# stcodeer/Frequency-wised_All-in-One_Image_Restoration_Model

Hardware: AMD Instinct MI355X
Metric: training images/sec @128x128 (higher is better)
Workload: dtype bf16; 1 GPU; BASELINE configs[1]: Uformer encoder+decoder (all_3_bands, L=3, freq MSA), denoise sigma=25, 128x128, phase-2 train step (fwd+bwd+Adam, DropPath on); per_gpu_batch=16, global_batch=16, parallelism=dp1, hip_graph=True

## Files before the change

### frequency-wised_all-in-one_image_restoration_model_amd/csrc/fw_elem.hip

```cpp
#include "fw_common.h"
#include <stdlib.h>

namespace {

constexpr int TPB = 256;
FW_DEV long gtid() { return (long)blockIdx.x * TPB + threadIdx.x; }
FW_DEV long gstride() { return (long)gridDim.x * TPB; }
static inline int grid_for(long n, int cap = 8192) { long g = (n + TPB - 1) / TPB; return (int)(g < 1 ? 1 : (g > cap ? cap : g)); }

template <typename T> FW_DEV void ldvec(const T* p, float* f) {
    unpack16<T>(*reinterpret_cast<const uint4*>(p), f);
}
template <typename T> FW_DEV void stvec(T* p, const float* f) { *reinterpret_cast<uint4*>(p) = pack16<T>(f); }
template <typename T> FW_DEV void ldvec4(const T* p, float* f);
template <> FW_SPEC void ldvec4<float>(const float* p, float* f) { unpack16<float>(*reinterpret_cast<const uint4*>(p), f); }
template <> FW_SPEC void ldvec4<bf16raw>(const bf16raw* p, float* f) {
    const uint2 v = *reinterpret_cast<const uint2*>(p);
    f[0] = __uint_as_float(v.x << 16); f[1] = __uint_as_float(v.x & 0xffff0000u);
    f[2] = __uint_as_float(v.y << 16); f[3] = __uint_as_float(v.y & 0xffff0000u);
}
template <typename T> FW_DEV void stvec4(T* p, const float* f);
template <> FW_SPEC void stvec4<float>(float* p, const float* f) { *reinterpret_cast<uint4*>(p) = pack16<float>(f); }
template <> FW_SPEC void stvec4<bf16raw>(bf16raw* p, const float* f) {
    *reinterpret_cast<uint2*>(p) = make_uint2(pack_bf2(f[0], f[1]), pack_bf2(f[2], f[3]));
}

template <typename T>
__global__ void cast_rows_kernel(const float* __restrict__ src, long lds_, T* __restrict__ dst, long ldd, long rows, int cols,
                                 const float* __restrict__ rowscale, int rps) {
    const int c4n = cols >> 2;
    for (long i = gtid(); i < rows * c4n; i += gstride()) {
        const long r = i / c4n; const int c = (int)(i % c4n) * 4;
        const f32x4 v = *reinterpret_cast<const f32x4*>(src + r * lds_ + c);
        const float s = rowscale ? rowscale[r / rps] : 1.f;
        T* d = dst + r * ldd + c;
        if (sizeof(T) == 4) *reinterpret_cast<f32x4*>(d) = v * s;
        else *reinterpret_cast<uint2*>(d) = make_uint2(pack_bf2(v[0] * s, v[1] * s), pack_bf2(v[2] * s, v[3] * s));
    }
}
__global__ void copy_rows_kernel(const float* __restrict__ src, long lds_, float* __restrict__ dst, long ldd, long rows, int cols, int acc) {
    const int c4n = cols >> 2;
    for (long i = gtid(); i < rows * c4n; i += gstride()) {
        const long r = i / c4n; const int c = (int)(i % c4n) * 4;
        f32x4 v = *reinterpret_cast<const f32x4*>(src + r * lds_ + c);
        if (acc) v += *reinterpret_cast<const f32x4*>(dst + r * ldd + c);
        *reinterpret_cast<f32x4*>(dst + r * ldd + c) = v;
    }
}
template <typename T>
__global__ void add_rows_kernel(const T* __restrict__ src, long lds_, T* __restrict__ dst, long ldd, long rows, int cols) {
    const int c4n = cols >> 2;
    for (long i = gtid(); i < rows * c4n; i += gstride()) {
        const long r = i / c4n; const int c = (int)(i % c4n) * 4;
        for (int e = 0; e < 4; ++e) {
// ... 917 lines not shown
        const int s = i & 3, l = (i >> 2) & 63, nt = (i >> 8) & 1, ch = i >> 9;
        const int k = ch * 16 + 4 * (l >> 4) + s, n = nt * 16 + (l & 15);
        sm[i] = (k < C && n < 27) ? w[((long)(n / 9) * C + k) * 9 + n % 9] : 0.f;
    }
    __syncthreads();
    const int l = lane_id(), wave = threadIdx.x >> 6;
    const EcTiles T(B, H, W);
    for (long t = blockIdx.x; t < T.n; t += gridDim.x) {
        long b; int y0, x0;
        T.at(t, b, y0, x0);
        for (int grp = wave; grp < (EC_PLANE + 15) / 16; grp += 4) {
            int r = grp * 16 + (l & 15); r = r < EC_PLANE ? r : EC_PLANE - 1;
            const int y = y0 + r / EC_PW - 1, x = x0 + r % EC_PW - 1;
            const bool ok = y >= 0 && y < H && x >= 0 && x < W;
            const int yc = y < 0 ? 0 : (y >= H ? H - 1 : y), xc = x < 0 ? 0 : (x >= W ? W - 1 : x);
            const float* row = fea + ((b * H + yc) * W + xc) * ldf;
            f32x4 acc0 = f32x4{0.f, 0.f, 0.f, 0.f}, acc1 = acc0;
            for (int c0 = 0; c0 < KC; c0 += 4) {
                uint4 af[4];
#pragma unroll
                for (int j = 0; j < 4; ++j) {
                    const int k = (c0 + j) * 16 + 4 * (l >> 4);
                    af[j] = *reinterpret_cast<const uint4*>(row + (k < C ? k : 0));
                }
#pragma unroll
                for (int j = 0; j < 4; ++j) {
                    const int k = (c0 + j) * 16 + 4 * (l >> 4);
                    if (!(ok && k < C)) af[j] = make_uint4(0u, 0u, 0u, 0u);
                    const int ch = c0 + j < KC ? c0 + j : KC - 1;
                    mma_chunk<float>(acc0, af[j], wl[(ch * 2 + 0) * 64 + l]);
                    mma_chunk<float>(acc1, af[j], wl[(ch * 2 + 1) * 64 + l]);
                }
            }
            float* pd = prod + (grp * 16 + 4 * (l >> 4)) * OP_PS + (l & 15);
#pragma unroll
            for (int rr = 0; rr < 4; ++rr) { pd[rr * OP_PS] = acc0[rr]; pd[rr * OP_PS + 16] = acc1[rr]; }
        }
        __syncthreads();
        for (int i = threadIdx.x; i < 3 * EC_PIX; i += 256) {
            const int co = i / EC_PIX, p = i % EC_PIX, ty = p / EC_TX, tx = p % EC_TX, y = y0 + ty, x = x0 + tx;
            const float* pp = prod + (ty * EC_PW + tx) * OP_PS + co * 9;
            const long po = ((b * 3 + co) * H + (y < H ? y : H - 1)) * W + (x < W ? x : W - 1);
            float s = bias[co] + (img ? img[po] : 0.f);
#pragma unroll
            for (int ky = 0; ky < 3; ++ky)
#pragma unroll
                for (int kx = 0; kx < 3; ++kx) s += pp[(ky * EC_PW + kx) * OP_PS + ky * 3 + kx];
            if (y < H && x < W) out[po] = s;
        }
        __syncthreads();
    }
}

__global__ void l1_loss_kernel(const float* __restrict__ a, const float* __restrict__ b, float* __restrict__ da, long n, float gscale,
                               float* __restrict__ loss) {
    float s = 0.f;
    for (long i = gtid(); i < n; i += gstride()) {
        const float d = a[i] - b[i];
        s += fabsf(d);
        if (da) da[i] = (d > 0.f ? 1.f : (d < 0.f ? -1.f : 0.f)) * gscale / n;
    }
    s = wave_sum(s);
    if (lane_id() == 0) atomicAdd(loss, s / n);
}
__global__ void ce0_loss_kernel(const float* __restrict__ logits, float* __restrict__ dlogits, int R, int N, float gscale, float* __restrict__ loss) {
    const int r = blockIdx.x;
    const float* x = logits + (long)r * N;
    float mx = -3.0e38f;
    for (int j = threadIdx.x; j < N; j += 64) mx = fmaxf(mx, x[j]);
    mx = wave_max(mx);
    float s = 0.f;
    for (int j = threadIdx.x; j < N; j += 64) s += __expf(x[j] - mx);
    s = wave_sum(s);
    const float lse = mx + __logf(s);
    if (dlogits)
        for (int j = threadIdx.x; j < N; j += 64) dlogits[(long)r * N + j] = (__expf(x[j] - lse) - (j == 0 ? 1.f : 0.f)) * gscale / R;
    if (threadIdx.x == 0) atomicAdd(loss, (lse - x[0]) / R);
}

__global__ void adam_tick_kernel(float* __restrict__ hyper, float b1, float b2) { hyper[1] *= b1; hyper[2] *= b2; hyper[3] += 1.f; }
template <typename T>
__global__ void adam_kernel(float* __restrict__ p, const float* __restrict__ g, float* __restrict__ m, float* __restrict__ v,
                            T* __restrict__ shadow, long n, const float* __restrict__ hyper, float b1, float b2, float eps) {
    const float lr = hyper[0], bc1 = 1.f - hyper[1], bc2_sqrt = sqrtf(1.f - hyper[2]);
    for (long i = gtid(); i < n; i += gstride()) {
        const float gi = g[i];
        const float mi = m[i] * b1 + gi * (1.f - b1);
        const float vi = v[i] * b2 + gi * gi * (1.f - b2);
        m[i] = mi; v[i] = vi;
        const float denom = sqrtf(vi) / bc2_sqrt + eps;
        const float pi = p[i] - (lr / bc1) * (mi / denom);
        p[i] = pi;
        if (shadow) TT<T>::st(shadow + i, pi);
    }
}
template <typename T>
__global__ void ema_kernel(float* __restrict__ pk, const float* __restrict__ pq, T* __restrict__ shadow, long n, float mom) {
    for (long i = gtid(); i < n; i += gstride()) {
        const float x = pk[i] * mom + pq[i] * (1.f - mom);
        pk[i] = x;
        if (shadow) TT<T>::st(shadow + i, x);
    }
}
template <typename T>
__global__ void lrelu_fwd_kernel(const float* __restrict__ x, T* __restrict__ y, long n, float slope) {
    for (long i = gtid(); i < n; i += gstride()) TT<T>::st(y + i, lrelu_f(x[i], slope));
}
template <typename T>
__global__ void lrelu_bwd_kernel(const T* __restrict__ dy, const float* __restrict__ x, float* __restrict__ dx, long n, float slope) {
    for (long i = gtid(); i < n; i += gstride()) dx[i] = TT<T>::ld(dy + i) * (x[i] > 0.f ? 1.f : slope);
}
__global__ __launch_bounds__(256) void slab_reduce_kernel(const float* __restrict__ slab, int nz, long n, long zstride, float* __restrict__ dst,
                                                          int accumulate, int zper, float* __restrict__ dst2, long off2, long n2) {
    __shared__ f32x4 red[3][64];
    const int lane = threadIdx.x & 63, zl = threadIdx.x >> 6;
    const long i4 = (long)blockIdx.x * 64 + lane;
    const long end = dst2 ? off2 + n2 : n;
    const bool live = i4 * 4 < end;
    const int z0 = blockIdx.y * zper, z1 = min(nz, z0 + zper);
    f32x4 s = f32x4{0.f, 0.f, 0.f, 0.f};
    if (live) {
        const float* p = slab + i4 * 4;
        int z = z0 + zl;
        for (; z + 12 < z1; z += 16) {
            const f32x4 a0 = *reinterpret_cast<const f32x4*>(p + (long)z * zstride);
            const f32x4 a1 = *reinterpret_cast<const f32x4*>(p + (long)(z + 4) * zstride);
            const f32x4 a2 = *reinterpret_cast<const f32x4*>(p + (long)(z + 8) * zstride);
            const f32x4 a3 = *reinterpret_cast<const f32x4*>(p + (long)(z + 12) * zstride);
            s += (a0 + a1) + (a2 + a3);
        }
        for (; z < z1; z += 4) s += *reinterpret_cast<const f32x4*>(p + (long)z * zstride);
    }
    if (zl > 0) red[zl - 1][lane] = s;
    __syncthreads();
    if (zl > 0 || !live) return;
    s += red[0][lane] + red[1][lane] + red[2][lane];
    for (int e = 0; e < 4; ++e) {
        const long i = i4 * 4 + e;
        float* d = nullptr;
        if (i < n) d = dst + i;
        else if (dst2 && i >= off2 && i < off2 + n2) d = dst2 + (i - off2);
        if (!d) continue;
        if (gridDim.y > 1) atomicAdd(d, s[e]);
        else if (accumulate) *d += s[e];
        else *d = s[e];
    }
}
__global__ __launch_bounds__(256) void slab_reduce_multi_kernel(const long long* __restrict__ tab, const long long* __restrict__ prefix, int num) {
    int lo = 0, hi = num;
    while (hi - lo > 1) {
        const int mid = (lo + hi) >> 1;
        if (prefix[mid] <= (long long)blockIdx.x) lo = mid; else hi = mid;
    }
    const long long* t = tab + (long)lo * 12;
// ... 241 lines not shown
    if (x_dtype == 1) hipLaunchKernelGGL((colsum_t_kernel<bf16raw>), dim3(grid), dim3(TPB), 0, ST, (const bf16raw*)x, ldx, out, rows, cols, rpb);
    else hipLaunchKernelGGL(colsum_kernel, dim3(grid), dim3(TPB), 0, ST, (const float*)x, ldx, out, rows, cols, rpb);
    FW_LAUNCH_RET();
}
#ifndef FW_EC_WGRAD_CAP
#define FW_EC_WGRAD_CAP 512
#endif
static inline int ec_grid(int B, int H, int W, int cap) {
    const long n = (long)B * ((H + EC_TY - 1) / EC_TY) * ((W + EC_TX - 1) / EC_TX);
    return (int)(n < cap ? n : cap);
}
static inline bool ec_al16(const void* p) { return ((uintptr_t)p & 15) == 0; }
constexpr int OP_PROD_BYTES = ((EC_PLANE + 15) / 16) * 16 * OP_PS * 4;
constexpr int OP_MAX_C = 896;
extern "C" int fw_inproj_fwd(const float* img, const float* w, const float* bias, float* out, long ldo, int B, int H, int W, int C,
                             float slope, void* stream) {
    FW_CHECK_ARG(img && w && bias && out && C % 4 == 0 && ldo % 4 == 0 && C > 0 && C <= 1024 && B > 0 && H > 0 && W > 0);
    FW_CHECK_ARG(ec_al16(out) && ec_al16(bias));
    hipLaunchKernelGGL(edge_conv3_rows_kernel<0>, dim3(ec_grid(B, H, W, 768)), dim3(TPB), 0, ST, img, w, bias, out, ldo, B, H, W, C, slope);
    FW_LAUNCH_RET();
}
extern "C" int fw_inproj_bwd(const float* img, const float* out, long ldo, const float* dy, long ldy, float* dw, float* db, int B,
                             int H, int W, int C, float slope, void* stream) {
    FW_CHECK_ARG(img && out && dy && dw && db && C > 0 && B > 0 && H > 0 && W > 0);
    const dim3 grid(ec_grid(B, H, W, FW_EC_WGRAD_CAP));
    const bool v4 = C % 4 == 0 && ldo % 4 == 0 && ldy % 4 == 0 && ec_al16(out) && ec_al16(dy);
    const int slice = v4 ? 1024 : 256;
    for (int c0 = 0; c0 < C; c0 += slice) {
        const int cs = C - c0 < slice ? C - c0 : slice;
        if (v4) hipLaunchKernelGGL((edge_conv3_wgrad_kernel<4, 0>), grid, dim3(TPB), 0, ST, img, dy + c0, ldy, out + c0, ldo, dw + (long)c0 * 27, db + c0, B, H, W, cs, slope);
        else hipLaunchKernelGGL((edge_conv3_wgrad_kernel<1, 0>), grid, dim3(TPB), 0, ST, img, dy + c0, ldy, out + c0, ldo, dw + (long)c0 * 27, db + c0, B, H, W, cs, slope);
    }
    FW_LAUNCH_RET();
}
extern "C" int fw_outproj_fwd(const float* fea, long ldf, const float* w, const float* bias, const float* img, float* out, int B,
                              int H, int W, int C, void* stream) {
    FW_CHECK_ARG(fea && w && bias && out && C % 4 == 0 && ldf % 4 == 0 && C > 0 && C <= OP_MAX_C && B > 0 && H > 0 && W > 0 && ec_al16(fea));
    const size_t lds = (size_t)((C + 15) / 16) * 2048 + OP_PROD_BYTES;
    FW_SET_LDS_ONCE(outproj_fwd_mfma_kernel, (OP_MAX_C / 16) * 2048 + OP_PROD_BYTES);
    hipLaunchKernelGGL(outproj_fwd_mfma_kernel, dim3(ec_grid(B, H, W, 512)), dim3(TPB), lds, ST, fea, ldf, w, bias, img, out, B, H, W, C);
    FW_LAUNCH_RET();
}
extern "C" int fw_outproj_bwd(const float* dout, const float* fea, long ldf, const float* w, float* dfea, long lddf, float* dw,
                              float* db, int B, int H, int W, int C, void* stream) {
    FW_CHECK_ARG(dout && fea && w && dfea && dw && db && C % 4 == 0 && ldf % 4 == 0 && lddf % 4 == 0 && C > 0 && C <= 1024 && B > 0 && H > 0 && W > 0);
    FW_CHECK_ARG(ec_al16(fea) && ec_al16(dfea));
    hipLaunchKernelGGL(edge_conv3_rows_kernel<1>, dim3(ec_grid(B, H, W, 768)), dim3(TPB), 0, ST, dout, w, (const float*)nullptr, dfea, lddf, B, H, W, C, 0.f);
    hipLaunchKernelGGL((edge_conv3_wgrad_kernel<4, 1>), dim3(ec_grid(B, H, W, FW_EC_WGRAD_CAP)), dim3(TPB), 0, ST, dout, fea, ldf, (const float*)nullptr, 0L, dw, db,
                       B, H, W, C, 0.f);
    FW_LAUNCH_RET();
}
extern "C" int fw_l1_loss(const float* a, const float* b, float* da, long n, float gscale, float* loss, void* stream) {
    FW_CHECK_ARG(a && b && loss && n > 0);
    hipLaunchKernelGGL(l1_loss_kernel, dim3(grid_for(n, 1024)), dim3(TPB), 0, ST, a, b, da, n, gscale, loss);
    FW_LAUNCH_RET();
}
extern "C" int fw_ce0_loss(const float* logits, float* dlogits, int R, int N, float gscale, float* loss, void* stream) {
    FW_CHECK_ARG(logits && loss && R > 0 && N > 0);
    hipLaunchKernelGGL(ce0_loss_kernel, dim3(R), dim3(64), 0, ST, logits, dlogits, R, N, gscale, loss);
    FW_LAUNCH_RET();
}
extern "C" int fw_adam_tick(float* hyper, float b1, float b2, void* stream) {
    FW_CHECK_ARG(hyper);
    hipLaunchKernelGGL(adam_tick_kernel, dim3(1), dim3(1), 0, ST, hyper, b1, b2);
    FW_LAUNCH_RET();
}
extern "C" int fw_adam(int shadow_dtype, float* p, const float* g, float* m, float* v, void* shadow, long n, const float* hyper,
                       float b1, float b2, float eps, void* stream) {
    FW_CHECK_ARG(p && g && m && v && hyper && n > 0);
    if (shadow_dtype == FW_DT_BF16 && shadow) LAUNCH((adam_kernel<bf16raw>), n, p, g, m, v, (bf16raw*)shadow, n, hyper, b1, b2, eps);
    LAUNCH((adam_kernel<float>), n, p, g, m, v, (float*)nullptr, n, hyper, b1, b2, eps);
}
extern "C" int fw_ema(int shadow_dtype, float* pk, const float* pq, void* shadow, long n, float momentum, void* stream) {
    FW_CHECK_ARG(pk && pq && n > 0);
    if (shadow_dtype == FW_DT_BF16 && shadow) LAUNCH((ema_kernel<bf16raw>), n, pk, pq, (bf16raw*)shadow, n, momentum);
    LAUNCH((ema_kernel<float>), n, pk, pq, (float*)nullptr, n, momentum);
}
extern "C" int fw_lrelu_fwd(int dtype, const float* x, void* y, long n, float slope, void* stream) {
    FW_CHECK_ARG(x && y && n > 0);
    if (dtype == FW_DT_BF16) LAUNCH((lrelu_fwd_kernel<bf16raw>), n, x, (bf16raw*)y, n, slope);
    LAUNCH((lrelu_fwd_kernel<float>), n, x, (float*)y, n, slope);
}
extern "C" int fw_lrelu_bwd(int dtype, const void* dy, const float* x, float* dx, long n, float slope, void* stream) {
    FW_CHECK_ARG(dy && x && dx && n > 0);
    if (dtype == FW_DT_BF16) LAUNCH((lrelu_bwd_kernel<bf16raw>), n, (const bf16raw*)dy, x, dx, n, slope);
    LAUNCH((lrelu_bwd_kernel<float>), n, (const float*)dy, x, dx, n, slope);
}
extern "C" int fw_slab_reduce(const float* slab, int nz, long n, long zstride, float* dst, int accumulate, float* dst2, long off2, long n2,
                              void* stream) {
    FW_CHECK_ARG(slab && dst && nz > 0 && n > 0 && zstride % 4 == 0 && ((uintptr_t)slab & 15) == 0);
    FW_CHECK_ARG(!dst2 || (off2 >= n && n2 > 0 && off2 + n2 <= zstride));
    const long end = dst2 ? off2 + n2 : n;
    const long gx = ((end + 3) / 4 + 63) / 64;
    int zper = nz;
    if (accumulate) {
        long splits = 1024 / gx;
        if (splits > nz / 8) splits = nz / 8;
        if (splits < 1) splits = 1;
        zper = (int)((nz + splits - 1) / splits);
    }
    dim3 grid((unsigned)gx, (unsigned)((nz + zper - 1) / zper));
    hipLaunchKernelGGL(slab_reduce_kernel, grid, dim3(256), 0, ST, slab, nz, n, zstride, dst, accumulate, zper, dst2, off2, n2);
    FW_LAUNCH_RET();
}
extern "C" int fw_slab_reduce_multi(const void* tab, const void* prefix, int num, long total_blocks, void* stream) {
    FW_CHECK_ARG(tab && prefix && num > 0 && total_blocks > 0 && total_blocks < (1L << 31));
    hipLaunchKernelGGL(slab_reduce_multi_kernel, dim3((unsigned)total_blocks), dim3(256), 0, ST, (const long long*)tab, (const long long*)prefix, num);
    FW_LAUNCH_RET();
}
extern "C" int fw_permute3_multi(const void* tab, const void* prefix, int num, long total_blocks, void* stream) {
    FW_CHECK_ARG(tab && prefix && num > 0 && total_blocks > 0 && total_blocks < (1L << 31));
    hipLaunchKernelGGL(permute3_multi_kernel, dim3((unsigned)total_blocks), dim3(256), 0, ST, (const long long*)tab, (const long long*)prefix, num);
    FW_LAUNCH_RET();
}
extern "C" int fw_fill(float* p, long n, float v, void* stream) {
    FW_CHECK_ARG(p && n > 0);
    LAUNCH(fill_kernel, n, p, n, v);
}
```

### frequency-wised_all-in-one_image_restoration_model_amd/csrc/fw_heads.hip

```cpp
#include "fw_common.h"

namespace {

template <int N> FW_DEV float block_sum(float v, float* red) {
    v = wave_sum(v);
    __syncthreads();
    if (lane_id() == 0) red[threadIdx.x >> 6] = v;
    __syncthreads();
    float s = 0.f;
    for (int i = 0; i < N / 64; ++i) s += red[i];
    return s;
}

constexpr int DFT_SL = 16, DFT_MAXN = 256;
__global__ __launch_bounds__(256) void dft2_fwd_kernel(const float* __restrict__ img, float* __restrict__ fr, float* __restrict__ fi, int N) {
    __shared__ float hr[DFT_SL * DFT_MAXN], hi[DFT_SL * DFT_MAXN], tc[DFT_MAXN], ts[DFT_MAXN];
    const int rows = N < DFT_SL ? N : DFT_SL;
    const int u0 = blockIdx.y * rows;
    const float* x = img + (size_t)blockIdx.x * N * N;
    for (int k = threadIdx.x; k < N; k += 256) { float sn, cs; sincospif(2.0f * k / N, &sn, &cs); tc[k] = cs; ts[k] = sn; }
    __syncthreads();
    for (int o = threadIdx.x; o < rows * N; o += 256) {
        const int u = u0 + o / N, xx = o % N;
        float ar = 0.f, ai = 0.f;
// ... 357 lines not shown
    float pos = 0.f;
    for (int c = threadIdx.x; c < ED; c += 256) {
        const float a = qq[c] * iq, bb = kk[c] * ik;
        sm[c] = a; khat[((size_t)l * B + b) * ED + c] = bb; pos += a * bb;
    }
    pos = block_sum<256>(pos, red);
    float* lg = logits + ((size_t)l * B + b) * (1 + K);
    if (threadIdx.x == 0) lg[0] = pos * invT;
    const float* Q = queue + (size_t)l * ED * K;
    for (int j = threadIdx.x; j < K; j += 256) {
        float s = 0.f;
        for (int c = 0; c < ED; ++c) s += sm[c] * Q[(size_t)c * K + j];
        lg[1 + j] = s * invT;
    }
}
__global__ __launch_bounds__(256) void moco_logits_bwd_kernel(const float* __restrict__ q, const float* __restrict__ khat, const float* __restrict__ queue,
                                                              const float* __restrict__ dlogits, float* __restrict__ dq, int B, int ED, int K, float invT) {
    __shared__ float red[4];
    const int l = blockIdx.x, b = blockIdx.y;
    const float* qq = q + ((size_t)l * B + b) * ED; const float* kh = khat + ((size_t)l * B + b) * ED;
    const float* dl = dlogits + ((size_t)l * B + b) * (1 + K);
    const float* Q = queue + (size_t)l * ED * K;
    float sq = 0.f;
    for (int c = threadIdx.x; c < ED; c += 256) sq += qq[c] * qq[c];
    sq = block_sum<256>(sq, red);
    const float nq = fmaxf(sqrtf(sq), 1e-12f), iq = 1.f / nq;
    float dot = 0.f;
    float loc[4];
    for (int t = 0; t < 4; ++t) {
        const int c = threadIdx.x + 256 * t;
        loc[t] = 0.f;
        if (c < ED) {
            float s = dl[0] * kh[c];
            for (int j = 0; j < K; ++j) s += dl[1 + j] * Q[(size_t)c * K + j];
            loc[t] = s * invT;
            dot += loc[t] * qq[c] * iq;
        }
    }
    dot = block_sum<256>(dot, red);
    for (int t = 0; t < 4; ++t) {
        const int c = threadIdx.x + 256 * t;
        if (c < ED) dq[((size_t)l * B + b) * ED + c] = (loc[t] - qq[c] * iq * dot) * iq;
    }
}
__global__ void moco_enqueue_kernel(float* __restrict__ queue, const float* __restrict__ khat, long long* __restrict__ ptr, int L, int B, int ED, int K) {
    const int p = (int)*ptr;
    for (int i = blockIdx.x * blockDim.x + threadIdx.x; i < L * B * ED; i += gridDim.x * blockDim.x) {
        const int c = i % ED, b = (i / ED) % B, l = i / (ED * B);
        queue[((size_t)l * ED + c) * K + p + b] = khat[i];
    }
}
__global__ void moco_ptr_kernel(long long* __restrict__ ptr, int B, int K) { *ptr = (*ptr + B) % K; }

constexpr int LFS_MAXT = 1024;
__global__ __launch_bounds__(256) void lfs_xbar_kernel(const float* __restrict__ inter, float* __restrict__ xbar, float* __restrict__ stats, int NT, int C, float eps) {
    __shared__ float mu[LFS_MAXT], rs[LFS_MAXT];
    const size_t blk = (size_t)blockIdx.x;
    const float* x = inter + blk * NT * C;
    const int w = threadIdx.x >> 6, l = lane_id();
    for (int t = w; t < NT; t += 4) {
        float s = 0.f;
        for (int c = l; c < C; c += 64) s += x[(size_t)t * C + c];
        const float m = wave_sum(s) / C;
        float q = 0.f;
        for (int c = l; c < C; c += 64) { const float d = x[(size_t)t * C + c] - m; q += d * d; }
        const float r = rsqrtf(wave_sum(q) / C + eps);
        if (l == 0) { mu[t] = m; rs[t] = r; stats[(blk * NT + t) * 2] = m; stats[(blk * NT + t) * 2 + 1] = r; }
    }
    __syncthreads();
    for (int c = threadIdx.x; c < C; c += 256) {
        float s = 0.f;
        for (int t = 0; t < NT; ++t) s += (x[(size_t)t * C + c] - mu[t]) * rs[t];
        xbar[blk * C + c] = s / NT;
    }
}
__global__ __launch_bounds__(256) void lfs_xbar_bwd_kernel(const float* __restrict__ inter, const float* __restrict__ stats, const float* __restrict__ dxbar,
                                                           float* __restrict__ dinter, int NT, int C) {
    __shared__ float red[4];
    const size_t blk = (size_t)blockIdx.x;
    const float* x = inter + blk * NT * C; float* dx = dinter + blk * NT * C;
    const float* g = dxbar + blk * C;
    float s = 0.f;
    for (int c = threadIdx.x; c < C; c += 256) s += g[c];
    const float m1 = block_sum<256>(s, red) / C / NT;
    const int w = threadIdx.x >> 6, l = lane_id();
    for (int t = w; t < NT; t += 4) {
        const float m = stats[(blk * NT + t) * 2], r = stats[(blk * NT + t) * 2 + 1];
        float q = 0.f;
        for (int c = l; c < C; c += 64) q += g[c] / NT * (x[(size_t)t * C + c] - m) * r;
        const float m2 = wave_sum(q) / C;
        for (int c = l; c < C; c += 64) {
            const float xh = (x[(size_t)t * C + c] - m) * r;
            dx[(size_t)t * C + c] += r * (g[c] / NT - m1 - xh * m2);
        }
    }
}

__global__ __launch_bounds__(64) void lfs_lambda_kernel(const float* __restrict__ xbar, const unsigned long long* __restrict__ ptab,
                                                        const int* __restrict__ heads, const long long* __restrict__ coef_off,
                                                        float* __restrict__ coef, float* __restrict__ save, int B, int C, int nb1) {
    __shared__ float u[16], s1[16], lam[2][16];
    const int blk = blockIdx.x, b = blockIdx.y, h = heads[blk], l = lane_id();
    for (int band = 0; band < nb1; ++band) {
        const unsigned long long* pt = ptab + ((size_t)blk * 2 + band) * 8;
        const float* lnw = (const float*)pt[0]; const float* lnb = (const float*)pt[1];
        const float* W = (const float*)pt[2]; const float* bl = (const float*)pt[3];
        const float* W1 = (const float*)pt[4]; const float* b1 = (const float*)pt[5];
        const float* W2 = (const float*)pt[6]; const float* b2 = (const float*)pt[7];
        const float* xb = xbar + ((size_t)band * B + b) * C;
        for (int hh = 0; hh < h; ++hh) {
            float s = 0.f;
            for (int c = l; c < C; c += 64) s += W[(size_t)hh * C + c] * (lnw[c] * xb[c] + lnb[c]);
            s = wave_sum(s);
            if (l == 0) u[hh] = s + bl[hh];
        }
        __syncthreads();
        float* sv = save + ((((size_t)blk * 2 + band) * B + b) * 16) * 3;
        if (l < h) {
            float a = b1[l];
            for (int j = 0; j < h; ++j) a += W1[l * h + j] * u[j];
            s1[l] = lrelu_f(a, 0.1f);
            sv[l * 3] = u[l]; sv[l * 3 + 1] = a; sv[l * 3 + 2] = s1[l];
        }
        __syncthreads();
        if (l < h) {
            float a = b2[l];
            for (int j = 0; j < h; ++j) a += W2[l * h + j] * s1[j];
            lam[band][l] = a;
        }
        __syncthreads();
    }
    if (l < h) {
        float* cf = coef + coef_off[blk] + ((size_t)b * h + l) * 3;
        if (nb1 == 2) { const float l1 = lam[0][l], l2 = lam[1][l]; cf[0] = 1.f + l2; cf[1] = -l2 * (1.f / 64.f); cf[2] = l1 - l2; }
        else { const float l1 = lam[0][l]; cf[0] = 1.f + l1; cf[1] = -l1 * (1.f / 64.f); cf[2] = 0.f; }
    }
}
__global__ __launch_bounds__(64) void lfs_lambda_bwd_kernel(const float* __restrict__ xbar, const unsigned long long* __restrict__ ptab,
                                                            const unsigned long long* __restrict__ gtab, const int* __restrict__ heads,
                                                            const long long* __restrict__ coef_off, const float* __restrict__ dcoef,
                                                            const float* __restrict__ save, float* __restrict__ dxbar, int B, int C, int nb1) {
    __shared__ float dl[16], da1[16], du[16];
    const int blk = blockIdx.x, b = blockIdx.y, h = heads[blk], l = lane_id();
    for (int band = 0; band < nb1; ++band) {
        const unsigned long long* pt = ptab + ((size_t)blk * 2 + band) * 8;
        const unsigned long long* gt = gtab + ((size_t)blk * 2 + band) * 8;
        const float* lnw = (const float*)pt[0]; const float* lnb = (const float*)pt[1];
// ... 83 lines not shown
    FW_LAUNCH_RET();
}

extern "C" int fw_bn_lrelu_gap_fwd(int dtype, const void* fea, const float* gamma, const float* beta, float* rmean, float* rvar,
                                   long long* nbt, float* part, float* saved, float* gap, int B, int ED, int P, int training,
                                   float eps, float momentum, float slope, void* stream) {
    FW_CHECK_ARG(fea && gamma && beta && rmean && rvar && gap && B > 0 && ED > 0 && P > 0 && (!training || (part && saved && nbt)));
    if (dtype == FW_DT_BF16) {
        if (training) hipLaunchKernelGGL((bn_stats_kernel<bf16raw>), dim3(ED, B), dim3(256), 0, ST, (const bf16raw*)fea, part, B, ED, P);
        hipLaunchKernelGGL((bn_apply_gap_kernel<bf16raw>), dim3(ED, B), dim3(256), 0, ST, (const bf16raw*)fea, part, gamma, beta, rmean, rvar, nbt,
                           gap, saved, B, ED, P, training, eps, momentum, slope);
    } else {
        if (training) hipLaunchKernelGGL((bn_stats_kernel<float>), dim3(ED, B), dim3(256), 0, ST, (const float*)fea, part, B, ED, P);
        hipLaunchKernelGGL((bn_apply_gap_kernel<float>), dim3(ED, B), dim3(256), 0, ST, (const float*)fea, part, gamma, beta, rmean, rvar, nbt, gap,
                           saved, B, ED, P, training, eps, momentum, slope);
    }
    FW_LAUNCH_RET();
}
extern "C" int fw_bn_lrelu_gap_bwd(int dtype, const void* fea, const float* gamma, const float* beta, const float* saved, const float* dgap,
                                   float* part2, void* dfea, float* dgamma, float* dbeta, int B, int ED, int P, float slope, void* stream) {
    FW_CHECK_ARG(fea && gamma && beta && saved && dgap && part2 && dfea && dgamma && dbeta);
    if (dtype == FW_DT_BF16) {
        hipLaunchKernelGGL((bn_bwd_stats_kernel<bf16raw>), dim3(ED, B), dim3(256), 0, ST, (const bf16raw*)fea, saved, gamma, beta, dgap, part2, B, ED, P, slope);
        hipLaunchKernelGGL((bn_bwd_apply_kernel<bf16raw>), dim3(ED, B), dim3(256), 0, ST, (const bf16raw*)fea, saved, gamma, beta, dgap, part2,
                           (bf16raw*)dfea, dgamma, dbeta, B, ED, P, slope);
    } else {
        hipLaunchKernelGGL((bn_bwd_stats_kernel<float>), dim3(ED, B), dim3(256), 0, ST, (const float*)fea, saved, gamma, beta, dgap, part2, B, ED, P, slope);
        hipLaunchKernelGGL((bn_bwd_apply_kernel<float>), dim3(ED, B), dim3(256), 0, ST, (const float*)fea, saved, gamma, beta, dgap, part2, (float*)dfea,
                           dgamma, dbeta, B, ED, P, slope);
    }
    FW_LAUNCH_RET();
}

extern "C" int fw_moco_logits(const float* q, const float* k, const float* queue, float* logits, float* khat, int L, int B, int ED, int K,
                              float invT, void* stream) {
    FW_CHECK_ARG(q && k && queue && logits && khat && L > 0 && B > 0 && ED > 0 && ED <= 1024 && K > 0);
    hipLaunchKernelGGL(moco_logits_kernel, dim3(L, B), dim3(256), (size_t)ED * 4, ST, q, k, queue, logits, khat, B, ED, K, invT);
    FW_LAUNCH_RET();
}
extern "C" int fw_moco_logits_bwd(const float* q, const float* khat, const float* queue, const float* dlogits, float* dq, int L, int B, int ED,
                                  int K, float invT, void* stream) {
    FW_CHECK_ARG(q && khat && queue && dlogits && dq && ED <= 1024);
    hipLaunchKernelGGL(moco_logits_bwd_kernel, dim3(L, B), dim3(256), 0, ST, q, khat, queue, dlogits, dq, B, ED, K, invT);
    FW_LAUNCH_RET();
}
extern "C" int fw_moco_enqueue(float* queue, const float* khat, long long* ptr, int L, int B, int ED, int K, void* stream) {
    FW_CHECK_ARG(queue && khat && ptr && K % B == 0);
    hipLaunchKernelGGL(moco_enqueue_kernel, dim3(fw_cdiv((long)L * B * ED, 256)), dim3(256), 0, ST, queue, khat, ptr, L, B, ED, K);
    hipLaunchKernelGGL(moco_ptr_kernel, dim3(1), dim3(1), 0, ST, ptr, B, K);
    FW_LAUNCH_RET();
}

extern "C" int fw_lfs_xbar(const float* inter, float* xbar, float* stats, int nb1, int B, int NT, int C, float eps, void* stream) {
    FW_CHECK_ARG(inter && xbar && stats && NT <= LFS_MAXT && NT > 0);
    hipLaunchKernelGGL(lfs_xbar_kernel, dim3(nb1 * B), dim3(256), 0, ST, inter, xbar, stats, NT, C, eps);
    FW_LAUNCH_RET();
}
extern "C" int fw_lfs_xbar_bwd(const float* inter, const float* stats, const float* dxbar, float* dinter, int nb1, int B, int NT, int C, void* stream) {
    FW_CHECK_ARG(inter && stats && dxbar && dinter);
    hipLaunchKernelGGL(lfs_xbar_bwd_kernel, dim3(nb1 * B), dim3(256), 0, ST, inter, stats, dxbar, dinter, NT, C);
    FW_LAUNCH_RET();
}
extern "C" int fw_lfs_lambda(const float* xbar, const unsigned long long* ptab, const int* heads, const long long* coef_off, float* coef,
                             float* save, int nblk, int B, int C, int nb1, void* stream) {
    FW_CHECK_ARG(xbar && ptab && heads && coef_off && coef && save && nblk > 0 && (nb1 == 1 || nb1 == 2));
    hipLaunchKernelGGL(lfs_lambda_kernel, dim3(nblk, B), dim3(64), 0, ST, xbar, ptab, heads, coef_off, coef, save, B, C, nb1);
    FW_LAUNCH_RET();
}
extern "C" int fw_lfs_lambda_bwd(const float* xbar, const unsigned long long* ptab, const unsigned long long* gtab, const int* heads,
                                 const long long* coef_off, const float* dcoef, const float* save, float* dxbar, int nblk, int B, int C,
                                 int nb1, void* stream) {
    FW_CHECK_ARG(xbar && ptab && gtab && heads && coef_off && dcoef && save && dxbar && (nb1 == 1 || nb1 == 2));
    hipLaunchKernelGGL(lfs_lambda_bwd_kernel, dim3(nblk, B), dim3(64), 0, ST, xbar, ptab, gtab, heads, coef_off, dcoef, save, dxbar, B, C, nb1);
    FW_LAUNCH_RET();
}
```

Baseline: 332.4 images/sec.

## Vectorize Adam/EMA/L1 kernels and widen parallelism of LFS xbar kernels

Adam, EMA and L1-loss kernels now use 16-byte vector loads and stores on an aligned body, with a scalar head and tail, two vectors per thread per iteration, and a block-level reduction before the atomic add. The LFS xbar forward kernel moves to 1024-thread blocks that process four rows at once and splits the channel reduction across a second grid dimension. The backward kernel gives one row per wave across a larger grid instead of looping over rows. The aim is to raise memory throughput in the optimizer and to fix under-occupied small grids. In exchange, the forward stats pass is recomputed redundantly in every channel slice.

```diff
diff --git a/frequency-wised_all-in-one_image_restoration_model_amd/csrc/fw_elem.hip b/frequency-wised_all-in-one_image_restoration_model_amd/csrc/fw_elem.hip
--- a/frequency-wised_all-in-one_image_restoration_model_amd/csrc/fw_elem.hip
+++ b/frequency-wised_all-in-one_image_restoration_model_amd/csrc/fw_elem.hip
@@ -1,5 +1,6 @@
 #include "fw_common.h"
 #include <stdlib.h>
+#include <initializer_list>
 
 namespace {
 
@@ -1023,16 +1024,56 @@
     }
 }
 
-__global__ void l1_loss_kernel(const float* __restrict__ a, const float* __restrict__ b, float* __restrict__ da, long n, float gscale,
-                               float* __restrict__ loss) {
+struct VecRange { long head, ng; };
+static inline VecRange vec_range(long n, const void* first, std::initializer_list<const void*> f32_ptrs, const void* bf16_ptr) {
+    const long head = (long)((16 - ((uintptr_t)first & 15)) & 15) / 4;
+    bool ok = ((uintptr_t)first & 3) == 0 && head < n;
+    for (const void* q : f32_ptrs) ok = ok && (((uintptr_t)q + head * 4) & 15) == 0;
+    if (bf16_ptr) ok = ok && (((uintptr_t)bf16_ptr + head * 2) & 7) == 0;
+    if (!ok) return VecRange{n, 0};
+    return VecRange{head, (n - head) >> 2};
+}
+static inline int vec_grid(long ng) { long g = (ng + 2 * TPB - 1) / (2 * TPB); return (int)(g < 1 ? 1 : (g > 2048 ? 2048 : g)); }
+FW_DEV long scalar_index(long k, long head, long ng) { return k < head ? k : k + 4 * ng; }
+FW_DEV f32x4 ld4(const float* p) { return *reinterpret_cast<const f32x4*>(p); }
+FW_DEV void st4(float* p, const f32x4& v) { *reinterpret_cast<f32x4*>(p) = v; }
+FW_DEV void st4_bf(bf16raw* p, const f32x4& v) { *reinterpret_cast<uint2*>(p) = make_uint2(pack_bf2(v[0], v[1]), pack_bf2(v[2], v[3])); }
+
+FW_DEV float l1_elem(float a, float b, float gn, float& s) {
+    const float d = a - b;
+    s += fabsf(d);
+    return (d > 0.f ? 1.f : (d < 0.f ? -1.f : 0.f)) * gn;
+}
+__global__ __launch_bounds__(256) void l1_loss_kernel(const float* __restrict__ a, const float* __restrict__ b, float* __restrict__ da, long n, long head,
+                                                      long ng, float gscale, float* __restrict__ loss) {
+    __shared__ float red[TPB / 64];
+    const float gn = gscale / n;
     float s = 0.f;
-    for (long i = gtid(); i < n; i += gstride()) {
-        const float d = a[i] - b[i];
-        s += fabsf(d);
-        if (da) da[i] = (d > 0.f ? 1.f : (d < 0.f ? -1.f : 0.f)) * gscale / n;
+    for (long i = gtid(); i < ng; i += 2 * gstride()) {
+        const bool two = i + gstride() < ng;
+        const long o0 = head + 4 * i, o1 = head + 4 * (two ? i + gstride() : i);
+        const f32x4 a0 = ld4(a + o0), b0 = ld4(b + o0), a1 = ld4(a + o1), b1 = ld4(b + o1);
+        f32x4 d0, d1;
+        float s1 = 0.f;
+#pragma unroll
+        for (int e = 0; e < 4; ++e) { d0[e] = l1_elem(a0[e], b0[e], gn, s); d1[e] = l1_elem(a1[e], b1[e], gn, s1); }
+        s += two ? s1 : 0.f;
+        if (da) { st4(da + o0, d0); st4(da + o1, d1); }
+    }
+    for (long k = gtid(); k < n - 4 * ng; k += gstride()) {
+        const long i = scalar_index(k, head, ng);
+        const float d = l1_elem(a[i], b[i], gn, s);
+        if (da) da[i] = d;
     }
     s = wave_sum(s);
-    if (lane_id() == 0) atomicAdd(loss, s / n);
+    if (lane_id() == 0) red[threadIdx.x >> 6] = s;
+    __syncthreads();
+    if (threadIdx.x == 0) {
+        float t = red[0];
+#pragma unroll
+        for (int w = 1; w < TPB / 64; ++w) t += red[w];
+        atomicAdd(loss, t / n);
+    }
 }
 __global__ void ce0_loss_kernel(const float* __restrict__ logits, float* __restrict__ dlogits, int R, int N, float gscale, float* __restrict__ loss) {
     const int r = blockIdx.x;
@@ -1050,27 +1091,65 @@
 }
 
 __global__ void adam_tick_kernel(float* __restrict__ hyper, float b1, float b2) { hyper[1] *= b1; hyper[2] *= b2; hyper[3] += 1.f; }
+FW_DEV void adam_elem(float& p, float gi, float& m, float& v, float b1, float b2, float eps, float step, float bc2_sqrt) {
+    const float mi = fmaf(gi, 1.f - b1, m * b1);
+    const float vi = fmaf(gi * gi, 1.f - b2, v * b2);
+    m = mi; v = vi;
+    const float denom = sqrtf(vi) / bc2_sqrt + eps;
+    p = fmaf(-step, mi / denom, p);
+}
+FW_DEV void adam_elem4(f32x4& p, const f32x4& g, f32x4& m, f32x4& v, float b1, float b2, float eps, float step, float bc2_sqrt) {
+#pragma unroll
+    for (int e = 0; e < 4; ++e) {
+        float pe = p[e], me = m[e], ve = v[e];
+        adam_elem(pe, g[e], me, ve, b1, b2, eps, step, bc2_sqrt);
+        p[e] = pe; m[e] = me; v[e] = ve;
+    }
+}
 template <typename T>
-__global__ void adam_kernel(float* __restrict__ p, const float* __restrict__ g, float* __restrict__ m, float* __restrict__ v,
-                            T* __restrict__ shadow, long n, const float* __restrict__ hyper, float b1, float b2, float eps) {
+__global__ __launch_bounds__(256) void adam_kernel(float* __restrict__ p, const float* __restrict__ g, float* __restrict__ m, float* __restrict__ v,
+                                                   T* __restrict__ shadow, long n, long head, long ng, const float* __restrict__ hyper, float b1, float b2,
+                                                   float eps) {
     const float lr = hyper[0], bc1 = 1.f - hyper[1], bc2_sqrt = sqrtf(1.f - hyper[2]);
-    for (long i = gtid(); i < n; i += gstride()) {
-        const float gi = g[i];
-        const float mi = m[i] * b1 + gi * (1.f - b1);
-        const float vi = v[i] * b2 + gi * gi * (1.f - b2);
-        m[i] = mi; v[i] = vi;
-        const float denom = sqrtf(vi) / bc2_sqrt + eps;
-        const float pi = p[i] - (lr / bc1) * (mi / denom);
-        p[i] = pi;
-        if (shadow) TT<T>::st(shadow + i, pi);
-    }
-}
+    const float step = lr / bc1;
+    for (long i = gtid(); i < ng; i += 2 * gstride()) {
+        const bool two = i + gstride() < ng;
+        const long o0 = head + 4 * i, o1 = head + 4 * (two ? i + gstride() : i);
+        const f32x4 g0 = ld4(g + o0), g1 = ld4(g + o1);
+        f32x4 m0 = ld4(m + o0), m1 = ld4(m + o1), v0 = ld4(v + o0), v1 = ld4(v + o1), p0 = ld4(p + o0), p1 = ld4(p + o1);
+        adam_elem4(p0, g0, m0, v0, b1, b2, eps, step, bc2_sqrt);
+        adam_elem4(p1, g1, m1, v1, b1, b2, eps, step, bc2_sqrt);
+        st4(m + o0, m0); st4(v + o0, v0); st4(p + o0, p0);
+        st4(m + o1, m1); st4(v + o1, v1); st4(p + o1, p1);
+        if constexpr (sizeof(T) == 2) { st4_bf(shadow + o0, p0); st4_bf(shadow + o1, p1); }
+    }
+    for (long k = gtid(); k < n - 4 * ng; k += gstride()) {
+        const long i = scalar_index(k, head, ng);
+        float pi = p[i], mi = m[i], vi = v[i];
+        adam_elem(pi, g[i], mi, vi, b1, b2, eps, step, bc2_sqrt);
+        m[i] = mi; v[i] = vi; p[i] = pi;
+        if constexpr (sizeof(T) == 2) TT<T>::st(shadow + i, pi);
+    }
+}
+FW_DEV float ema_elem(float k, float q, float mom) { return fmaf(k, mom, q * (1.f - mom)); }
 template <typename T>
-__global__ void ema_kernel(float* __restrict__ pk, const float* __restrict__ pq, T* __restrict__ shadow, long n, float mom) {
-    for (long i = gtid(); i < n; i += gstride()) {
-        const float x = pk[i] * mom + pq[i] * (1.f - mom);
+__global__ __launch_bounds__(256) void ema_kernel(float* __restrict__ pk, const float* __restrict__ pq, T* __restrict__ shadow, long n, long head, long ng,
+                                                  float mom) {
+    for (long i = gtid(); i < ng; i += 2 * gstride()) {
+        const bool two = i + gstride() < ng;
+        const long o0 = head + 4 * i, o1 = head + 4 * (two ? i + gstride() : i);
+        const f32x4 q0 = ld4(pq + o0), q1 = ld4(pq + o1);
+        f32x4 k0 = ld4(pk + o0), k1 = ld4(pk + o1);
+#pragma unroll
+        for (int e = 0; e < 4; ++e) { k0[e] = ema_elem(k0[e], q0[e], mom); k1[e] = ema_elem(k1[e], q1[e], mom); }
+        st4(pk + o0, k0); st4(pk + o1, k1);
+        if constexpr (sizeof(T) == 2) { st4_bf(shadow + o0, k0); st4_bf(shadow + o1, k1); }
+    }
+    for (long k = gtid(); k < n - 4 * ng; k += gstride()) {
+        const long i = scalar_index(k, head, ng);
+        const float x = ema_elem(pk[i], pq[i], mom);
         pk[i] = x;
-        if (shadow) TT<T>::st(shadow + i, x);
+        if constexpr (sizeof(T) == 2) TT<T>::st(shadow + i, x);
     }
 }
 template <typename T>
@@ -1418,7 +1497,8 @@
 }
 extern "C" int fw_l1_loss(const float* a, const float* b, float* da, long n, float gscale, float* loss, void* stream) {
     FW_CHECK_ARG(a && b && loss && n > 0);
-    hipLaunchKernelGGL(l1_loss_kernel, dim3(grid_for(n, 1024)), dim3(TPB), 0, ST, a, b, da, n, gscale, loss);
+    const VecRange r = vec_range(n, a, {a, b, da ? (const void*)da : (const void*)a}, nullptr);
+    hipLaunchKernelGGL(l1_loss_kernel, dim3(r.ng ? vec_grid(r.ng) : grid_for(n, 1024)), dim3(TPB), 0, ST, a, b, da, n, r.head, r.ng, gscale, loss);
     FW_LAUNCH_RET();
 }
 extern "C" int fw_ce0_loss(const float* logits, float* dlogits, int R, int N, float gscale, float* loss, void* stream) {
@@ -1434,13 +1514,21 @@
 extern "C" int fw_adam(int shadow_dtype, float* p, const float* g, float* m, float* v, void* shadow, long n, const float* hyper,
                        float b1, float b2, float eps, void* stream) {
     FW_CHECK_ARG(p && g && m && v && hyper && n > 0);
-    if (shadow_dtype == FW_DT_BF16 && shadow) LAUNCH((adam_kernel<bf16raw>), n, p, g, m, v, (bf16raw*)shadow, n, hyper, b1, b2, eps);
-    LAUNCH((adam_kernel<float>), n, p, g, m, v, (float*)nullptr, n, hyper, b1, b2, eps);
+    const bool sh = shadow_dtype == FW_DT_BF16 && shadow;
+    const VecRange r = vec_range(n, p, {p, g, m, v}, sh ? shadow : nullptr);
+    const dim3 grid(r.ng ? vec_grid(r.ng) : grid_for(n));
+    if (sh) hipLaunchKernelGGL((adam_kernel<bf16raw>), grid, dim3(TPB), 0, ST, p, g, m, v, (bf16raw*)shadow, n, r.head, r.ng, hyper, b1, b2, eps);
+    else hipLaunchKernelGGL((adam_kernel<float>), grid, dim3(TPB), 0, ST, p, g, m, v, (float*)nullptr, n, r.head, r.ng, hyper, b1, b2, eps);
+    FW_LAUNCH_RET();
 }
 extern "C" int fw_ema(int shadow_dtype, float* pk, const float* pq, void* shadow, long n, float momentum, void* stream) {
     FW_CHECK_ARG(pk && pq && n > 0);
-    if (shadow_dtype == FW_DT_BF16 && shadow) LAUNCH((ema_kernel<bf16raw>), n, pk, pq, (bf16raw*)shadow, n, momentum);
-    LAUNCH((ema_kernel<float>), n, pk, pq, (float*)nullptr, n, momentum);
+    const bool sh = shadow_dtype == FW_DT_BF16 && shadow;
+    const VecRange r = vec_range(n, pk, {pk, pq}, sh ? shadow : nullptr);
+    const dim3 grid(r.ng ? vec_grid(r.ng) : grid_for(n));
+    if (sh) hipLaunchKernelGGL((ema_kernel<bf16raw>), grid, dim3(TPB), 0, ST, pk, pq, (bf16raw*)shadow, n, r.head, r.ng, momentum);
+    else hipLaunchKernelGGL((ema_kernel<float>), grid, dim3(TPB), 0, ST, pk, pq, (float*)nullptr, n, r.head, r.ng, momentum);
+    FW_LAUNCH_RET();
 }
 extern "C" int fw_lrelu_fwd(int dtype, const float* x, void* y, long n, float slope, void* stream) {
     FW_CHECK_ARG(x && y && n > 0);
diff --git a/frequency-wised_all-in-one_image_restoration_model_amd/csrc/fw_heads.hip b/frequency-wised_all-in-one_image_restoration_model_amd/csrc/fw_heads.hip
--- a/frequency-wised_all-in-one_image_restoration_model_amd/csrc/fw_heads.hip
+++ b/frequency-wised_all-in-one_image_restoration_model_amd/csrc/fw_heads.hip
@@ -433,23 +433,44 @@
 }
 __global__ void moco_ptr_kernel(long long* __restrict__ ptr, int B, int K) { *ptr = (*ptr + B) % K; }
 
-constexpr int LFS_MAXT = 1024;
-__global__ __launch_bounds__(256) void lfs_xbar_kernel(const float* __restrict__ inter, float* __restrict__ xbar, float* __restrict__ stats, int NT, int C, float eps) {
+constexpr int LFS_MAXT = 1024, LFS_XT = 1024, LFS_XR = 4, LFS_XS = 8;
+static inline int lfs_xslices(int C) { const int s = C / 32; return s < 1 ? 1 : (s > LFS_XS ? LFS_XS : s); }
+__global__ __launch_bounds__(LFS_XT) void lfs_xbar_kernel(const float* __restrict__ inter, float* __restrict__ xbar, float* __restrict__ stats, int NT, int C, float eps) {
     __shared__ float mu[LFS_MAXT], rs[LFS_MAXT];
     const size_t blk = (size_t)blockIdx.x;
     const float* x = inter + blk * NT * C;
     const int w = threadIdx.x >> 6, l = lane_id();
-    for (int t = w; t < NT; t += 4) {
-        float s = 0.f;
-        for (int c = l; c < C; c += 64) s += x[(size_t)t * C + c];
-        const float m = wave_sum(s) / C;
-        float q = 0.f;
-        for (int c = l; c < C; c += 64) { const float d = x[(size_t)t * C + c] - m; q += d * d; }
-        const float r = rsqrtf(wave_sum(q) / C + eps);
-        if (l == 0) { mu[t] = m; rs[t] = r; stats[(blk * NT + t) * 2] = m; stats[(blk * NT + t) * 2 + 1] = r; }
+    constexpr int NW = LFS_XT / 64;
+    for (int t0 = w; t0 < NT; t0 += NW * LFS_XR) {
+        const float* row[LFS_XR];
+        float s[LFS_XR], q[LFS_XR], m[LFS_XR];
+#pragma unroll
+        for (int r = 0; r < LFS_XR; ++r) {
+            const int t = t0 + r * NW;
+            row[r] = x + (size_t)(t < NT ? t : NT - 1) * C;
+            s[r] = 0.f; q[r] = 0.f;
+        }
+        for (int c = l; c < C; c += 64)
+#pragma unroll
+            for (int r = 0; r < LFS_XR; ++r) s[r] += row[r][c];
+#pragma unroll
+        for (int r = 0; r < LFS_XR; ++r) m[r] = wave_sum(s[r]) / C;
+        for (int c = l; c < C; c += 64)
+#pragma unroll
+            for (int r = 0; r < LFS_XR; ++r) { const float d = row[r][c] - m[r]; q[r] += d * d; }
+#pragma unroll
+        for (int r = 0; r < LFS_XR; ++r) {
+            const int t = t0 + r * NW;
+            const float rr = rsqrtf(wave_sum(q[r]) / C + eps);
+            if (l == 0 && t < NT) {
+                mu[t] = m[r]; rs[t] = rr;
+                if (blockIdx.y == 0) { stats[(blk * NT + t) * 2] = m[r]; stats[(blk * NT + t) * 2 + 1] = rr; }
+            }
+        }
     }
     __syncthreads();
-    for (int c = threadIdx.x; c < C; c += 256) {
+    const int cw = (C + gridDim.y - 1) / gridDim.y, c0 = blockIdx.y * cw;
+    for (int c = c0 + threadIdx.x; c < c0 + cw && c < C; c += LFS_XT) {
         float s = 0.f;
         for (int t = 0; t < NT; ++t) s += (x[(size_t)t * C + c] - mu[t]) * rs[t];
         xbar[blk * C + c] = s / NT;
@@ -465,15 +486,15 @@
     for (int c = threadIdx.x; c < C; c += 256) s += g[c];
     const float m1 = block_sum<256>(s, red) / C / NT;
     const int w = threadIdx.x >> 6, l = lane_id();
-    for (int t = w; t < NT; t += 4) {
-        const float m = stats[(blk * NT + t) * 2], r = stats[(blk * NT + t) * 2 + 1];
-        float q = 0.f;
-        for (int c = l; c < C; c += 64) q += g[c] / NT * (x[(size_t)t * C + c] - m) * r;
-        const float m2 = wave_sum(q) / C;
-        for (int c = l; c < C; c += 64) {
-            const float xh = (x[(size_t)t * C + c] - m) * r;
-            dx[(size_t)t * C + c] += r * (g[c] / NT - m1 - xh * m2);
-        }
+    const int t = blockIdx.y * 4 + w;
+    if (t >= NT) return;
+    const float m = stats[(blk * NT + t) * 2], r = stats[(blk * NT + t) * 2 + 1];
+    float q = 0.f;
+    for (int c = l; c < C; c += 64) q += g[c] / NT * (x[(size_t)t * C + c] - m) * r;
+    const float m2 = wave_sum(q) / C;
+    for (int c = l; c < C; c += 64) {
+        const float xh = (x[(size_t)t * C + c] - m) * r;
+        dx[(size_t)t * C + c] += r * (g[c] / NT - m1 - xh * m2);
     }
 }
 
@@ -663,13 +684,13 @@
 }
 
 extern "C" int fw_lfs_xbar(const float* inter, float* xbar, float* stats, int nb1, int B, int NT, int C, float eps, void* stream) {
-    FW_CHECK_ARG(inter && xbar && stats && NT <= LFS_MAXT && NT > 0);
-    hipLaunchKernelGGL(lfs_xbar_kernel, dim3(nb1 * B), dim3(256), 0, ST, inter, xbar, stats, NT, C, eps);
+    FW_CHECK_ARG(inter && xbar && stats && NT <= LFS_MAXT && NT > 0 && C > 0 && nb1 > 0 && B > 0);
+    hipLaunchKernelGGL(lfs_xbar_kernel, dim3(nb1 * B, lfs_xslices(C)), dim3(LFS_XT), 0, ST, inter, xbar, stats, NT, C, eps);
     FW_LAUNCH_RET();
 }
 extern "C" int fw_lfs_xbar_bwd(const float* inter, const float* stats, const float* dxbar, float* dinter, int nb1, int B, int NT, int C, void* stream) {
-    FW_CHECK_ARG(inter && stats && dxbar && dinter);
-    hipLaunchKernelGGL(lfs_xbar_bwd_kernel, dim3(nb1 * B), dim3(256), 0, ST, inter, stats, dxbar, dinter, NT, C);
+    FW_CHECK_ARG(inter && stats && dxbar && dinter && NT > 0 && C > 0 && nb1 > 0 && B > 0);
+    hipLaunchKernelGGL(lfs_xbar_bwd_kernel, dim3(nb1 * B, (NT + 3) / 4), dim3(256), 0, ST, inter, stats, dxbar, dinter, NT, C);
     FW_LAUNCH_RET();
 }
 extern "C" int fw_lfs_lambda(const float* xbar, const unsigned long long* ptab, const int* heads, const long long* coef_off, float* coef,
```

Measured after the change: 333.5 images/sec (median of 6 runs). No clear change (+0.3%).
